# althonos/pyhmmer

Measured on AMD Instinct MI355X. Metric: GCUPS (DP cells/s) + seqs/s for hmmsearch, Pfam-A vs proteome, 1/2/4/8 GPUs, higher is better.
Workload: dtype u8/i16 filters (MSV, Viterbi), f32 Forward/Backward

## Files before the change

pyhmmer_amd/csrc/p7x_device.hpp:

```cpp
#pragma once
#include "p7x_internal.hpp"
#include "p7x_devmem.hpp"
#include <hip/hip_runtime.h>
#include <map>
#include <memory>
#include <mutex>

namespace p7x {

constexpr int kMaxL      = 100000;
constexpr int kTabRows   = 32;
constexpr int kNegPad    = -512;

#define P7X_HIP(call)                                                                          \
  do { hipError_t e_ = (call); if (e_ != hipSuccess) {                                         \
    p7x::set_error(std::string(#call) + ": " + hipGetErrorString(e_)); return e_ == hipErrorOutOfMemory ? P7X_EMEM : P7X_EDEVICE; } } while (0)

struct LengthTables {
  uint8_t *tjb = nullptr;
  int16_t *xwmove = nullptr;
  float   *null1 = nullptr;
  double  *logtab = nullptr;
};

struct DeviceCtx {
  int device = -1;
  hipStream_t stream = nullptr;
  hipStream_t stream2 = nullptr;
  LengthTables lt;
  int num_cu = 256;
  std::mutex mu;
  std::mutex msv_mu;
  std::mutex lt_scan_mu;
  static constexpr int kLtStreams = 4;
  hipStream_t lt_stream[kLtStreams]{};
  int lt_next = 0;
  hipEvent_t msv_done[2] = { nullptr, nullptr };
  int msv_last = -1;
  std::mutex slab_mu;
  std::multimap<size_t, void *> slab_free;
  size_t slab_free_bytes = 0;
  size_t slab_obtained_bytes = 0;
  static constexpr int kWsSets = 4, kWsSide = 7;
  hipStream_t ws_main[kWsSets]{};
  hipStream_t ws_side[kWsSets][kWsSide]{};
  std::vector<hipStream_t> ws_spacers;
  int ws_set_users[kWsSets]{};
};
int get_ctx(int device, DeviceCtx **out);
int create_tail_stream(DeviceCtx *ctx, bool high_priority, hipStream_t *out);

struct DevProfile {
  int device = -1;
  int M = 0, Kp = 0;
  int msvR = 0, msvK = 0, msvS = 0;
  uint32_t *msv_tab = nullptr;
  int16_t *msvw_emis = nullptr;
  uint32_t *msvw_pk = nullptr;
  int msvwC = 0, msvw_rows = kTabRows;
  int vitC = 0, Mpad = 0;
  int16_t *vit_trans = nullptr;
  int16_t *vit_emis = nullptr;
  int vitpkT = 0, vitpkP = 0;
  uint32_t *vitpk_trans = nullptr, *vitpk_emis = nullptr;
  float *fwd_trans = nullptr;
  float *fwd_emis = nullptr;
  int fwdgT = 0, fwdgC = 0;
  float *fwdg_trans = nullptr, *fwdg_emis = nullptr;
  float *bias_eo = nullptr;
  std::shared_ptr<DeviceBuf> shared;
};

int get_dev_profile(const p7x_oprofile *om, DeviceCtx *ctx, DevProfile **out);
int get_dev_profiles(const p7x_oprofile *const *oms, int n, DeviceCtx *ctx, DevProfile **out, int nthreads);
void free_dev_profile(DevProfile *d);

struct EnvelopeScorer;
struct EnsembleRunner;
}
struct p7x_seqdb;
#include <memory>
namespace p7x {
struct LongTargetWindowRegions;
int device_regions_of_all(const p7x_oprofile *om, const p7x_seqdb *db, std::vector<LongTargetWindowRegions> &out);
std::unique_ptr<EnvelopeScorer> make_device_envelope_scorer(DeviceCtx *ctx, const p7x_seqdb *db, float oa_guard);
std::unique_ptr<EnvelopeScorer> make_device_align_scorer(DeviceCtx *ctx, const p7x_seqdb *db, float oa_guard);
size_t align_budget_bytes();
std::unique_ptr<EnsembleRunner> make_device_ensemble_runner(DeviceCtx *ctx, const p7x_seqdb *db, float guard);

}

struct p7x_seqdb {
  int device = -1;
  int abc_type = 0, Kp = 0;
  int64_t n = 0;
  int64_t nres = 0;
  int64_t nslots = 0;
  int64_t ngroups = 0;
  std::vector<int32_t> h_len;
  std::vector<int32_t> h_order;
  std::vector<int64_t> h_off;
  std::vector<uint8_t> h_dsq;
  int64_t vit_long_slots = 0;
  std::vector<int32_t> h_grp_len;
  std::vector<int64_t> h_grp_suffix;
  uint8_t *d_dsq = nullptr;
  int64_t *d_slot_off = nullptr;
  int32_t *d_slot_len = nullptr;
  uint4   *d_tiles = nullptr;
  int64_t *d_grp_off = nullptr;
  int32_t *d_grp_nblk = nullptr;
  int64_t tile_u4 = 0;
  p7x::DeviceBuf slab;
};
```

pyhmmer_amd/csrc/p7x_devimage.hip:

```cpp
#include "p7x_device.hpp"
#include "p7x_kernels.hpp"
#include "p7x_host.hpp"
#include <cstring>
#include <memory>

namespace p7x {

static void chunk_transpose_fill(int M, int C, std::vector<int> &pos_of_node)
{
  pos_of_node.assign(M + 1, -1);
  for (int k = 1; k <= M; ++k) { const int z = (k - 1) / C, c = (k - 1) % C; pos_of_node[k] = c * 64 + z; }
}

void free_dev_profile(DevProfile *d)
{
  delete d;
}

struct DevCache { std::mutex mu; std::vector<DevProfile *> per_device; };

struct ImageStage { int device = -1; PinnedBuf pinned; hipStream_t stream = nullptr; };

struct HostImage {
  std::vector<char> bytes;
  std::vector<std::pair<void **, size_t>> fix;
  template <typename T, typename F>
  void add(F **field, const std::vector<T> &v)
  {
    const size_t off = bytes.size(), n = v.size() * sizeof(T);
    bytes.resize(((off + n + 255) / 256) * 256);
    std::memcpy(bytes.data() + off, v.data(), n);
    fix.emplace_back(reinterpret_cast<void **>(field), off);
  }
};

static void build_host_image(const Profile &p, DevProfile *d, HostImage &img)
{
  d->msvR = msv_pick(p.M, &d->msvK);
  if (d->msvR > 0) {
    d->msvS = msv_stride(d->msvR, d->msvK);
    std::vector<uint32_t> tab;
    msv_build_tables(p, d->msvR, d->msvK, tab);
    img.add(&d->msv_tab, tab);
  }
  d->vitC = vit_pick_C(p.M);
  if (d->vitC > 0) {
    const int C = d->vitC, Mpad = 64 * C, nrows = p.Kp + 1;
    d->Mpad = Mpad;
    std::vector<int> pos;
    chunk_transpose_fill(p.M, C, pos);
    std::vector<int16_t> vt((size_t) Mpad * 8, -32768), ve((size_t) nrows * Mpad, -32768);
    std::vector<float> ft((size_t) Mpad * 8, 0.0f), fe((size_t) nrows * Mpad, 0.0f);
    for (int k = 1; k <= p.M; ++k) {
      for (int t = 0; t < NTRANS; ++t) {
        vt[(size_t) pos[k] * 8 + t] = p.tw[(size_t) t * (p.M + 1) + k];
        ft[(size_t) pos[k] * 8 + t] = p.tf[(size_t) t * (p.M + 1) + k];
      }
      for (int x = 0; x < p.Kp; ++x) {
        ve[(size_t) x * Mpad + pos[k]] = p.rw[(size_t) x * (p.M + 1) + k];
        fe[(size_t) x * Mpad + pos[k]] = p.rf_[(size_t) x * (p.M + 1) + k];
      }
    }
    {
      std::vector<int16_t> me((size_t) kTabRows * Mpad, (int16_t) kNegPad);
      for (int k = 1; k <= p.M; ++k)
        for (int x = 0; x < p.Kp; ++x) me[(size_t) x * Mpad + pos[k]] = (int16_t) ((int) p.bias_b - (int) p.rb[(size_t) x * (p.M + 1) + k]);
      img.add(&d->msvw_emis, me);
      d->msvwC = C; d->msvw_rows = kTabRows;
      int Cp = 0;
      if ((d->msvR <= 0 || d->msvK >= 8) && C % 4 == 0 && C <= 32) Cp = C;
      else if (d->msvR <= 0 && C > 32 && p.M <= 2560 && p.Kp + 1 <= 30) { Cp = p.M <= 2304 ? 36 : 40; d->msvwC = Cp; d->msvw_rows = p.Kp + 1; }
      if (Cp > 0) {
        const int P2 = Cp / 4, rows = d->msvw_rows;
        std::vector<uint32_t> pk((size_t) rows * P2 * 64 * 2);
        auto em = [&](int x, int k) -> uint32_t { return (uint32_t) (uint16_t) (int16_t) ((x < p.Kp && k <= p.M) ? (int) p.bias_b - (int) p.rb[(size_t) x * (p.M + 1) + k] : kNegPad); };
        for (int x = 0; x < rows; ++x)
          for (int j2 = 0; j2 < P2; ++j2)
            for (int z = 0; z < 64; ++z)
              for (int h = 0; h < 2; ++h) {
                const int k = z * Cp + 2 * (2 * j2 + h) + 1;
                pk[(((size_t) x * P2 + j2) * 64 + z) * 2 + h] = em(x, k) | (em(x, k + 1) << 16);
              }
        img.add(&d->msvw_pk, pk);
      }
    }
    img.add(&d->vit_trans, vt);
    img.add(&d->vit_emis, ve);
    img.add(&d->fwd_trans, ft);
    img.add(&d->fwd_emis, fe);
    int gT = 0, gC = 0;
    if (fwdg_pick(p.M, d->vitC, &gT, &gC)) {
      std::vector<float> gt, ge;
      fwdg_build_tables(p, gT, gC, gt, ge);
      d->fwdgT = gT; d->fwdgC = gC;
      img.add(&d->fwdg_trans, gt);
      img.add(&d->fwdg_emis, ge);
    }
  }
  {
    int T = 0, P = 0;
    if (vitpk_pick(p.M, &T, &P)) {
      std::vector<uint32_t> tt, te;
      vitpk_build_tables(p, T, P, tt, te);
      d->vitpkT = T; d->vitpkP = P;
      img.add(&d->vitpk_trans, tt);
      img.add(&d->vitpk_emis, te);
    }
  }
  {
    const Alphabet &abc = Alphabet::get(p.abc_type);
    std::vector<float> eo((size_t) kTabRows * 2, 1.0f);
    for (int x = 0; x < p.K; ++x) { eo[x * 2 + 0] = p.bgf[x] / p.bgf[x]; eo[x * 2 + 1] = p.compo[x] / p.bgf[x]; }
    for (int x = p.K + 1; x <= p.Kp - 3; ++x)
      for (int s = 0; s < 2; ++s) {
        float e = 0.0f, den = 0.0f;
        for (int y = 0; y < p.K; ++y) if (abc.degen[x][y]) { e += (s == 0 ? p.bgf[y] : p.compo[y]); den += p.bgf[y]; }
        eo[x * 2 + s] = den > 0.0f ? e / den : 0.0f;
      }
    img.add(&d->bias_eo, eo);
  }
}

int get_dev_profiles(const p7x_oprofile *const *oms, int n, DeviceCtx *ctx, DevProfile **out, int nthreads)
{
  std::vector<int> missing;
  for (int i = 0; i < n; ++i) {
    out[i] = nullptr;
    auto *cache = static_cast<DevCache *>(oms[i]->dev_cache);
    std::lock_guard<std::mutex> lk(cache->mu);
    for (DevProfile *d : cache->per_device) if (d->device == ctx->device) { out[i] = d; break; }
    if (!out[i]) missing.push_back(i);
  }
  if (missing.empty()) return P7X_OK;
  const int nm = (int) missing.size();
  std::vector<std::unique_ptr<DevProfile>> fresh((size_t) nm);
  std::vector<HostImage> imgs((size_t) nm);
  auto build = [&](int z) {
    const Profile &p = oms[missing[(size_t) z]]->p;
    auto d = std::make_unique<DevProfile>();
    d->device = ctx->device; d->M = p.M; d->Kp = p.Kp;
    build_host_image(p, d.get(), imgs[(size_t) z]);
    fresh[(size_t) z] = std::move(d);
  };
  if (nm >= 4) host_parallel_for(nm, nthreads, build); else for (int z = 0; z < nm; ++z) build(z);
  std::vector<size_t> off((size_t) nm + 1, 0);
  for (int z = 0; z < nm; ++z) off[(size_t) z + 1] = off[(size_t) z] + imgs[(size_t) z].bytes.size();
  const size_t total = off[(size_t) nm];
  auto stage_lease = LeasePool<ImageStage>::instance().lease(ctx->device, [](const ImageStage &, const ImageStage *b) { return !b; });
  ImageStage &stg = *stage_lease;
  int st = P7X_OK;
  if ((st = stg.pinned.reserve(total, (size_t) 1 << 20)) != P7X_OK) return st;
  if (stg.stream == nullptr) P7X_HIP(hipStreamCreateWithFlags(&stg.stream, hipStreamNonBlocking));
  auto shared = std::make_shared<DeviceBuf>();
  if ((st = shared->reserve(ctx, total)) != P7X_OK) return st;
  char *const pinned = stg.pinned.as<char>(), *const slab = shared->as<char>();
  auto place = [&](int z) {
    const HostImage &img = imgs[(size_t) z];
    std::memcpy(pinned + off[(size_t) z], img.bytes.data(), img.bytes.size());
    for (const auto &f : img.fix) *f.first = slab + off[(size_t) z] + f.second;
    fresh[(size_t) z]->shared = shared;
  };
  if (nm >= 4) host_parallel_for(nm, nthreads, place); else for (int z = 0; z < nm; ++z) place(z);
  if (hipMemcpyAsync(slab, pinned, total, hipMemcpyHostToDevice, stg.stream) != hipSuccess ||
      hipStreamSynchronize(stg.stream) != hipSuccess) {
    set_error("uploading the profiles' device images failed");
    return P7X_EDEVICE;
  }
  for (int z = 0; z < nm; ++z) {
    const int i = missing[(size_t) z];
    auto *cache = static_cast<DevCache *>(oms[i]->dev_cache);
    std::lock_guard<std::mutex> lk(cache->mu);
    for (DevProfile *d : cache->per_device) if (d->device == ctx->device) { out[i] = d; break; }
    if (!out[i]) { out[i] = fresh[(size_t) z].get(); cache->per_device.push_back(fresh[(size_t) z].release()); }
  }
  return P7X_OK;
}

int get_dev_profile(const p7x_oprofile *om, DeviceCtx *ctx, DevProfile **out) { return get_dev_profiles(&om, 1, ctx, out, 1); }

}

using namespace p7x;

extern "C" {

void p7x_oprofile_destroy(p7x_oprofile *om)
// ... 14 lines not shown
```

pyhmmer_amd/csrc/p7x_kernels.hpp:

```cpp
#pragma once
#include <type_traits>
#include "p7x_device.hpp"

namespace p7x {

struct ArgRef { const void *base; uint32_t stride; };
#if defined(__HIPCC__)
template <class A> __device__ __forceinline__ A load_args(const ArgRef r)
{
#if defined(__HIP_DEVICE_COMPILE__)
  typedef const __attribute__((address_space(4))) A *cptr;
  return *(cptr) (unsigned long long) (static_cast<const char *>(r.base) + (size_t) blockIdx.y * r.stride);
#else
  return *reinterpret_cast<const A *>(static_cast<const char *>(r.base) + (size_t) blockIdx.y * r.stride);
#endif
}
#endif
template <class A> struct ArgRun {
  const A *host = nullptr; const void *dev = nullptr; uint32_t stride = 0; int n = 0;
  const A &at(int i) const { return *reinterpret_cast<const A *>(reinterpret_cast<const char *>(host) + (size_t) i * stride); }
  ArgRef ref() const { return ArgRef{ dev, stride }; }
};
inline unsigned lane_grid(long want, long resident, int nlanes)
{
  (void) nlanes;
  if (want > resident) want = resident;
  return (unsigned) (want < 1 ? 1 : want);
}

inline unsigned lane_grid_pull(long want, long resident, int nlanes, bool old_rule)
{
  if (old_rule || nlanes < 32) return lane_grid(want, resident, nlanes);
  long b = (2 * resident + nlanes - 1) / nlanes;
  if (b > resident) b = resident;
  if (b > want) b = want;
  return (unsigned) (b < 1 ? 1 : b);
}

struct MsvArgs {
  const uint32_t *tab;
  const uint4 *tiles;
  const int64_t *grp_off;
  const int32_t *grp_nblk;
  const int32_t *slot_len;
  const uint8_t *tjb_tab;
  int ngroups;
  int group_first;
  int base, bias, tec, tbm;
  int *counter;
  int16_t *out_xJ;
  int *amb_count; int *amb_groups; int *counter2;
  const int *group_list; const int *group_count;
  int R;
};
int  msv_pick(int M, int *K);
int  msv_stride(int R, int K);
void msv_build_tables(const Profile &p, int R, int K, std::vector<uint32_t> &out);
int  msv_launch(int R, int K, const ArgRun<MsvArgs> &main, const ArgRun<MsvArgs> *amb, int num_cu, hipStream_t st);
constexpr int kMsvTiers = 6;
int  msv_tier(int R, int K);
int  msv_tier_launch(int tier, const ArgRun<MsvArgs> &main, int num_cu, hipStream_t st);
int  msv_exact_launch(int R, int K, const ArgRun<MsvArgs> &amb, int num_cu, hipStream_t st);

#define P7X_NODE_TIERS(X) X(1) X(2) X(3) X(4) X(5) X(6) X(8) X(10) X(12) X(16) X(20) X(24) X(32) X(48) X(64) X(96) X(128)
template <class F> int node_tier_dispatch(int C, const char *too_long, F &&f)
{
  switch (C) {
#define P7X_TIER_CASE(CC) case CC: return f(std::integral_constant<int, CC>());
    P7X_NODE_TIERS(P7X_TIER_CASE)
#undef P7X_TIER_CASE
    default: set_error(too_long); return P7X_EINVAL;
  }
}
struct WaveSeqArgs {
  int M, C;
  const void *trans;
  const void *emis;
  const uint8_t *dsq;
  const int64_t *slot_off;
  const int32_t *slot_len;
  const int32_t *list;
  int nlist;
  const int *nlist_ptr;
  const int *abort_flag;
  int nrows;
  int *counter;
  const int16_t *xwmove_tab; int base_w, xw_e, ddbound;
  int32_t *out_xC;
  const int *lt_thresh;
  int *lt_nrec; int *lt_rec; int lt_cap;
  float xf_e_move, xf_e_loop;
  float *out_sc;
  float *xmx;
  const int64_t *xmx_off;
  const float *fwd_xmx;
};
int vit_pick_C(int M);
int vit_launch(const ArgRun<WaveSeqArgs> &a, int num_cu, hipStream_t st);
int fwd_launch(const ArgRun<WaveSeqArgs> &a, int num_cu, hipStream_t st);
bool fwdg_pick(int M, int vitC, int *T, int *C);
int fwdg_launch(const ArgRun<WaveSeqArgs> &a, int num_cu, hipStream_t st);
void fwdg_build_tables(const Profile &p, int T, int C, std::vector<float> &trans, std::vector<float> &emis);
int bck_launch(const ArgRun<WaveSeqArgs> &a, int num_cu, hipStream_t st);

struct MsvWaveArgs {
  int C, nrows;
  const void *emis;
  const void *emis_pk;
  const uint8_t *dsq; const int64_t *slot_off; const int32_t *slot_len; const uint8_t *tjb_tab;
  int nslots, base, bias, tec, tbm;
  int16_t *out_xJ;
};
int msv_wave_launch(const ArgRun<MsvWaveArgs> &a, int num_cu, hipStream_t st);

struct VitPkArgs {
  const void *trans, *emis;
  const uint8_t *dsq; const int64_t *slot_off; const int32_t *slot_len;
  const int32_t *list; int nlist; const int *nlist_ptr;
  const int *nskip_ptr;
  int nrows;
  const int16_t *xwmove_tab; int base_w, xw_e, ddbound;
  int32_t *out_xC;
};
bool vitpk_pick(int M, int *T, int *P);
void vitpk_build_tables(const Profile &p, int T, int P, std::vector<uint32_t> &trans, std::vector<uint32_t> &emis);
int  vitpk_launch(int T, int P, const ArgRun<VitPkArgs> &a, int num_cu, hipStream_t st);

struct EnvArgs {
  int M, C, K, nrows;
  const void *trans;
  const void *emis;
  const uint8_t *dsq;
  float nj, xf_e_move, xf_e_loop;
  int nenv;
  const int64_t *env_sq;
  const int32_t *env_len;
  const int32_t *env_L;
  const int32_t *order;
  int *cursor;
  float *work; int64_t work_stride; int Lmax;
  int nblocks, slab_base;
  float *out_sc;
  const float *env_emis;
  long long env_emis_stride;
  float *out_orig;
  float oa_guard;
  int32_t *out_status;
  float *out_null2;
  const int64_t *tr_off;
  uint32_t *tr_a; int32_t *tr_i; float *tr_pp;
  int32_t *tr_n;
};
constexpr int env_waves(int C) { return C >= 8 ? 4 : 8; }
enum class EnvMode { Envelope, LongTarget, Align };
inline size_t env_work_floats(int C, int Lmax)
{
  const size_t rows = (size_t) Lmax + 1, Mpad = (size_t) 64 * C;
  size_t f = 2 * rows * Mpad + rows * (6 + 6 + 5 + 3 + 1);
  f += (rows * Mpad + 1) / 2;
  return (f + 63) & ~(size_t) 63;
}
int env_max_blocks(EnvMode mode, int C, int nrows, int num_cu, int *nblocks);
int env_launch(EnvMode mode, const ArgRun<EnvArgs> &a, hipStream_t st);
__host__ __device__ inline float align_pp_guard(int M) { return 1.0e-5f + 2.5e-9f * (float) M; }
__host__ __device__ inline float align_pp_band(int M) { return 0.5f - 10.0f * align_pp_guard(M); }
int align_max_blocks(int C, int nrows, int num_cu, int *nblocks);
int align_launch(const ArgRun<EnvArgs> &a, hipStream_t st);

struct ChoiceCell; struct ChoiceRow;
struct EnsRegion {
  int64_t sq;
  int64_t cell0;
  int64_t row0;
  int64_t dom0;
  int32_t Lr, L;
  int32_t job, dom_cap;
};
struct EnsJob {
  int M, C, K, Kp, nrows, Q;
  const void *trans, *emis;
  const float *rft;
  const uint8_t *degen;
  int reg_first, nreg;
};
struct EnsArgs {
  const EnsJob *jobs; const EnsRegion *regions; int nregions;
  const uint8_t *dsq;
  ChoiceCell *cells; float2 *md; ChoiceRow *rows;
  uint32_t seed_x;
  int nsamples;
  float *n2acc;
  int32_t *dom;
  int32_t *out_ndom; int32_t *out_status;
  int lds_bytes;
  uint32_t guard;
};

struct SsvLongArgs {
  const uint32_t *tab4q;
  const uint32_t *tab_full;
  const uint8_t *dsq;
  const uint8_t *comp;
  int pair_slack;
  const long long *chunk_list;
  long long L;
  int M, Kp;
  int chunk_len;
  long long chunks_per_strand, nchunks;
// ... 12 lines not shown
```

pyhmmer_amd/csrc/p7x_pipeline.hip:

```cpp
#include "p7x_wave.hpp"
#include "p7x_host.hpp"
#include <atomic>
#include <chrono>
#include <cmath>
#include <cstdlib>
#include <cstring>
#include <memory>
#include <string>

namespace p7x {

struct StageBufs {
  int16_t *xJ;
  float *usc, *filtersc, *vfsc, *fwdsc;
  int32_t *xC;
  float *fwd_by_item;
  int32_t *list_bias, *list_vit, *list_fwd, *list_fin;
  uint8_t *stage;
  int *counters;
};

struct StageParams {
  double F1, F2, F3;
  double F3_near;
// ... 556 lines not shown
static ListEstimates estimate_lists(const p7x_pipeline_cfg &cfg, int64_t nslots)
{
  auto est = [&](double f, double slack, int floor_) {
    const double v = cfg.do_max ? (double) nslots : std::min<double>((double) nslots, (double) nslots * f * slack + floor_);
    return (int) std::min<double>(v, (double) INT_MAX);
  };
  ListEstimates e;
  e.bias = est(cfg.F1, 2.0, 1024); e.vit = e.bias;
  e.fwd = est(cfg.F2, 8.0, 512);
  e.fin = est(cfg.F3, 50.0, 1024);
  return e;
}

static WaveSeqArgs ws_args(const Profile &p, const DevProfile *dp, const p7x_seqdb *db, DeviceCtx *ctx)
{
  WaveSeqArgs a{};
  a.M = p.M; a.C = dp->vitC; a.nrows = p.Kp + 1;
  a.dsq = db->d_dsq; a.slot_off = db->d_slot_off; a.slot_len = db->d_slot_len;
  a.xwmove_tab = ctx->lt.xwmove; a.base_w = p.base_w; a.xw_e = p.xw[XE][MOVE]; a.ddbound = p.ddbound_w;
  a.xf_e_move = p.xf[XE][MOVE]; a.xf_e_loop = p.xf[XE][LOOP];
  return a;
}

static bool msv_exact_only() { return debug_opt(OPT_MSV_EXACT) > 0; }
static bool vit_wave_only() { return debug_opt(OPT_VIT_WAVE) > 0; }
static bool device_clustered(int host_threads)
{
  const int forced = debug_opt(OPT_DEVICE_CLUSTERED);
  if (forced >= 0) return forced != 0;
  const int threads = host_threads > 0 ? std::min(host_threads, tophits_usable_cpus()) : tophits_usable_cpus();
  return threads < 12;
}

static bool small_block(const p7x_seqdb *db, const DeviceCtx *ctx, int nlanes)
{
  return debug_opt(OPT_SMALL_BLOCK) != 0 && db->ngroups * (int64_t) nlanes <= (int64_t) ctx->num_cu * 4;
}

static int long_groups(const p7x_seqdb *db, const DeviceCtx *ctx, int nlanes)
{
  if (debug_opt(OPT_MSV_LONG_GROUPS) == 0 || db->ngroups < 2) return 0;
  const int64_t resident = (int64_t) ctx->num_cu * 4 * 3;
  const int64_t G = db->ngroups;
  int64_t g = 0;
  while (g < G / 2 && (int64_t) db->h_grp_len[(size_t) g] * resident > (int64_t) nlanes * db->h_grp_suffix[(size_t) g]) ++g;
  return (int) g;
}

static void fill_msv_args(LaneArgs &la, const Profile &p, const DevProfile *dp, const p7x_seqdb *db, DeviceCtx *ctx, const StageBufs &b,
                          int nlong = 0)
{
  MsvWaveArgs w{};
  w.C = dp->msvwC; w.nrows = dp->msvw_rows; w.emis = dp->msvw_emis; w.emis_pk = dp->msvw_pk; w.dsq = db->d_dsq; w.slot_off = db->d_slot_off; w.slot_len = db->d_slot_len;
  w.tjb_tab = ctx->lt.tjb; w.nslots = (int) db->nslots; w.base = p.base_b; w.bias = p.bias_b; w.tec = p.tec_b; w.tbm = p.tbm_b;
  w.out_xJ = b.xJ;
  if (nlong > 0) w.nslots = (int) std::min<int64_t>((int64_t) nlong * 64, db->nslots);
  la.msvw = w;
  MsvArgs a{};
  a.group_first = nlong;
  a.tab = dp->msv_tab; a.tiles = db->d_tiles; a.grp_off = db->d_grp_off; a.grp_nblk = db->d_grp_nblk;
  a.slot_len = db->d_slot_len; a.tjb_tab = ctx->lt.tjb; a.ngroups = (int) db->ngroups;
  a.base = p.base_b; a.bias = p.bias_b; a.tec = p.tec_b; a.tbm = p.tbm_b;
  a.counter = &b.counters[0]; a.out_xJ = b.xJ;
  a.amb_count = &b.counters[10]; a.counter2 = &b.counters[11];
  a.amb_groups = msv_exact_only() ? nullptr : b.list_fin;
  a.R = dp->msvR;
  la.msv = a;
  MsvArgs x = a;
  x.group_list = a.amb_groups; x.group_count = a.amb_count; x.counter = a.counter2; x.amb_groups = nullptr;
  la.msv_amb = x;
}

static void fill_vit_args(LaneArgs &la, const Profile &p, const DevProfile *dp, const p7x_seqdb *db, DeviceCtx *ctx,
                          const int32_t *list, int nlist, const int *nlist_ptr, int32_t *out_xC,
                          const int *nlong_ptr = nullptr, int nlong_bound = 0)
{
  WaveSeqArgs w = ws_args(p, dp, db, ctx);
  w.trans = dp->vit_trans; w.emis = dp->vit_emis; w.list = list; w.nlist = nlist; w.nlist_ptr = nlist_ptr; w.out_xC = out_xC;
  if (nlong_ptr) { w.nlist_ptr = nlong_ptr; w.nlist = nlong_bound; }
  la.vit = w;
  VitPkArgs a{};
  a.trans = dp->vitpk_trans; a.emis = dp->vitpk_emis; a.dsq = db->d_dsq; a.slot_off = db->d_slot_off; a.slot_len = db->d_slot_len;
  a.list = list; a.nlist = nlist; a.nlist_ptr = nlist_ptr; a.nskip_ptr = nlong_ptr; a.nrows = p.Kp + 1;
  a.xwmove_tab = ctx->lt.xwmove; a.base_w = p.base_w; a.xw_e = p.xw[XE][MOVE]; a.ddbound = p.ddbound_w;
  a.out_xC = out_xC;
  la.vitpk = a;
}

template <class A> static ArgRun<A> lane_run(const Workspace *ws, A LaneArgs::*member, int first, int n)
{
  ArgRun<A> r;
  r.host = &(ws->h_args.as<LaneArgs>()[first].*member);
  r.dev = reinterpret_cast<const char *>(ws->d_args.as<LaneArgs>() + first) + (reinterpret_cast<const char *>(r.host) - reinterpret_cast<const char *>(ws->h_args.as<LaneArgs>() + first));
  r.stride = (uint32_t) sizeof(LaneArgs); r.n = n;
  return r;
}

struct LaneModel { const p7x_oprofile *om = nullptr; DevProfile *dp = nullptr; };

static int upload_args(Workspace *ws, int first, int n, hipStream_t s)
{
  P7X_HIP(hipMemcpyAsync(ws->d_args.as<LaneArgs>() + first, ws->h_args.as<LaneArgs>() + first, (size_t) n * sizeof(LaneArgs), hipMemcpyHostToDevice, s));
  return P7X_OK;
}

struct LaneClass { int first = 0, n = 0; long msv_key = 0, vit_key = 0; int C = 0; int nlong = 0; int64_t vit_long = 0; };

static long msv_key_of(const DevProfile *dp, bool small)
{
  return (dp->msvR <= 0 || small) ? -(long) dp->msvwC : (long) (dp->msvK * 1000 + dp->msvR);
}
static long vit_key_of(const DevProfile *dp, bool small)
{
  return (dp->vitpkT > 0 && !vit_wave_only() && !small) ? (long) (dp->vitpkT * 256 + dp->vitpkP) : -(long) dp->vitC;
}

static int lane_classes(const std::vector<LaneModel> &lm, const p7x_seqdb *db, const DeviceCtx *ctx, std::vector<LaneClass> &out)
{
  const int nl = (int) lm.size();
  const bool small = small_block(db, ctx, nl);
  const int nlong = small ? 0 : long_groups(db, ctx, nl);
  out.clear();
  for (int l = 0; l < nl; ++l) {
    const DevProfile *dp = lm[l].dp;
    if ((dp->msvR <= 0 || small) && !dp->msvw_emis) { set_error("model too long for the MSV kernels (M > 8192)"); return P7X_EINVAL; }
    LaneClass c; c.first = l; c.n = 1; c.msv_key = msv_key_of(dp, small); c.vit_key = vit_key_of(dp, small); c.C = dp->vitC;
    c.nlong = (c.msv_key >= 0 && dp->msvw_emis) ? nlong : 0;
    c.vit_long = c.vit_key >= 0 ? db->vit_long_slots : 0;
    if (!out.empty() && out.back().msv_key == c.msv_key && out.back().vit_key == c.vit_key && out.back().C == c.C) out.back().n++;
    else out.push_back(c);
  }
  return P7X_OK;
}

static int class_msv(const LaneClass &c, const std::vector<LaneModel> &lm, DeviceCtx *ctx, Workspace *ws, hipStream_t stream)
{
  if (c.msv_key < 0) return msv_wave_launch(lane_run(ws, &LaneArgs::msvw, c.first, c.n), ctx->num_cu, stream);
  if (c.nlong > 0) {
    const int st = msv_wave_launch(lane_run(ws, &LaneArgs::msvw, c.first, c.n), ctx->num_cu, stream);
    if (st != P7X_OK) return st;
  }
  const ArgRun<MsvArgs> amb = lane_run(ws, &LaneArgs::msv_amb, c.first, c.n);
  return msv_launch(lm[c.first].dp->msvR, lm[c.first].dp->msvK, lane_run(ws, &LaneArgs::msv, c.first, c.n), msv_exact_only() ? nullptr : &amb, ctx->num_cu, stream);
}

static int class_msv_rest(const LaneClass &c, const std::vector<LaneModel> &lm, DeviceCtx *ctx, Workspace *ws, hipStream_t stream)
{
  if (c.nlong > 0) {
    const int st = msv_wave_launch(lane_run(ws, &LaneArgs::msvw, c.first, c.n), ctx->num_cu, stream);
    if (st != P7X_OK) return st;
  }
  return msv_exact_launch(lm[c.first].dp->msvR, lm[c.first].dp->msvK, lane_run(ws, &LaneArgs::msv_amb, c.first, c.n), ctx->num_cu, stream);
}
static bool msv_tiers_enabled() { return !msv_exact_only() && debug_opt(OPT_MSV_F16) != 0 && debug_opt(OPT_MSV_TIERS) != 0; }

static int class_viterbi(const LaneClass &c, const std::vector<LaneModel> &lm, DeviceCtx *ctx, Workspace *ws, hipStream_t s)
{
  if (c.vit_key < 0) return vit_launch(lane_run(ws, &LaneArgs::vit, c.first, c.n), ctx->num_cu, s);
  if (c.vit_long > 0) {
    const int st = vit_launch(lane_run(ws, &LaneArgs::vit, c.first, c.n), ctx->num_cu, s);
    if (st != P7X_OK) return st;
  }
  return vitpk_launch(lm[c.first].dp->vitpkT, lm[c.first].dp->vitpkP, lane_run(ws, &LaneArgs::vitpk, c.first, c.n), ctx->num_cu, s);
}

static int class_wave(const LaneClass &c, Workspace *ws, WaveSeqArgs LaneArgs::*member, bool backward, DeviceCtx *ctx, hipStream_t s)
{
// ... 1086 lines not shown
```

pyhmmer_amd/csrc/p7x_vitpk.hip:

```cpp
#include <map>
#include "p7x_wave.hpp"
#include <mutex>

namespace p7x {

namespace {

typedef short s2v __attribute__((ext_vector_type(2)));
__device__ __forceinline__ s2v as_s2v(uint32_t u) { return __builtin_bit_cast(s2v, u); }
__device__ __forceinline__ uint32_t as_u(s2v v) { return __builtin_bit_cast(uint32_t, v); }
__device__ __forceinline__ uint32_t pk_adds(uint32_t a, uint32_t b) { return as_u(__builtin_elementwise_add_sat(as_s2v(a), as_s2v(b))); }
__device__ __forceinline__ uint32_t pk_max(uint32_t a, uint32_t b) { return as_u(__builtin_elementwise_max(as_s2v(a), as_s2v(b))); }
__device__ __forceinline__ uint32_t splat16(int v) { const uint32_t w = (uint32_t) v & 0xffffu; return w | (w << 16); }
__device__ __forceinline__ int lo_of(uint32_t w) { return (int) (short) (w & 0xffffu); }
__device__ __forceinline__ int hi_of(uint32_t w) { return (int) (short) (w >> 16); }

constexpr uint32_t kNeg2 = 0x80008000u;
constexpr int vitpk_rowq(int T, int P)
{
  const int n = ((P + 3) / 4) * T;
  return T == 8 ? ((n & 15) == 8 ? n : n + 8) : n;
}

#define P7X_DPP_U(v, ctrl) ((uint32_t) __builtin_amdgcn_update_dpp((int) kNeg2, (int) (v), (ctrl), 0xf, 0xf, false))

template <int T>
__device__ __forceinline__ int group_max(uint32_t v)
{
  v = pk_max(v, P7X_DPP_U(v, 0xB1));
  v = pk_max(v, P7X_DPP_U(v, 0x4E));
  v = pk_max(v, P7X_DPP_U(v, 0x141));
  if constexpr (T == 16) v = pk_max(v, P7X_DPP_U(v, 0x140));
  return max(lo_of(v), hi_of(v));
}

}

struct RowState { int xN, xB, xJ, xC; bool overflow; };

template <int T>
__device__ __forceinline__ uint32_t stripe_shift(uint32_t r, bool first)
{
  const uint32_t prev = P7X_DPP_U(r, 0x138);
  const uint32_t last = P7X_DPP_U(r, T == 8 ? 0x141 : 0x140);
  return first ? ((last << 16) | 0x8000u) : prev;
}

template <int T, int P>
__device__ __forceinline__ void vit_row(const VitPkArgs &a, const uint4 *tral, const uint4 *trbl, const uint4 *er, bool first,
                                        bool active, int xwm, const uint32_t (&mi)[P], const uint32_t (&ii)[P],
                                        const uint32_t (&di)[P], uint32_t (&mo_)[P], uint32_t (&io_)[P], uint32_t (&do_)[P],
                                        const uint32_t (&tdd)[P], RowState &rs)
{
  constexpr int PS = (P + 3) & ~3;
  const uint32_t xBv = splat16(rs.xB);
  uint32_t mp = stripe_shift<T>(mi[P - 1], first), ip = stripe_shift<T>(ii[P - 1], first), dp = stripe_shift<T>(di[P - 1], first);
  uint32_t xEv = kNeg2, dmaxv = kNeg2, dcv = kNeg2;
#pragma unroll
  for (int j4 = 0; j4 < PS; j4 += 4) {
    const uint4 e4 = er[(j4 / 4) * T];
    const uint32_t ev[4] = { e4.x, e4.y, e4.z, e4.w };
#pragma unroll
    for (int jj = 0; jj < 4; ++jj) {
      const int q = j4 + jj;
      if (q < P) {
        const uint4 ta = tral[q * T], tb = trbl[q * T];
        const uint32_t a0 = pk_adds(xBv, ta.x), a1 = pk_adds(mp, ta.y), a2 = pk_adds(ip, ta.z), a3 = pk_adds(dp, ta.w);
        uint32_t sv = pk_max(pk_max(a0, a1), pk_max(a2, a3));
        sv = pk_adds(sv, ev[jj]);
        xEv = pk_max(xEv, sv);
        mo_[q] = sv;
        if (q > 0) do_[q] = dcv;
        dcv = pk_adds(sv, tb.x);
        dmaxv = pk_max(dmaxv, dcv);
        io_[q] = pk_max(pk_adds(mi[q], tb.y), pk_adds(ii[q], tb.z));
        mp = mi[q]; ip = ii[q]; dp = di[q];
      }
    }
    asm volatile("" ::: "memory");
  }
  do_[0] = stripe_shift<T>(dcv, first);
  const int xE = group_max<T>(xEv);
  const int Dmax = group_max<T>(dmaxv);
  if (active) {
    if (xE >= 32767) rs.overflow = true;
    rs.xC = max(rs.xC, xE + a.xw_e);
    rs.xJ = max(rs.xJ, xE + a.xw_e);
    rs.xB = max(rs.xJ + xwm, rs.xN + xwm);
  }
  const bool trig = active && (Dmax + a.ddbound > rs.xB);
#ifdef P7X_VITPK_NO_CLOSURE
  if (false) {
#else
  if (__any(trig)) {
#endif
    int pass = 0;
    bool more;
    do {
#pragma unroll
      for (int q = 1; q < P; ++q) do_[q] = pk_max(do_[q], pk_adds(do_[q - 1], tdd[q - 1]));
      uint32_t c = stripe_shift<T>(pk_adds(do_[P - 1], tdd[P - 1]), first);
      if (!trig) c = kNeg2;
      const uint32_t d0 = pk_max(do_[0], c);
      const bool changed = d0 != do_[0];
      do_[0] = d0;
      more = __any(changed) && ++pass < 2 * T;
    } while (more);
  }
}

template <int T, int P>
__global__ void __launch_bounds__(256) vitpk_kernel(const ArgRef ref)
{
  constexpr int G = 64 / T;
  const VitPkArgs a = load_args<VitPkArgs>(ref);
  const int nlist = a.nlist_ptr ? *a.nlist_ptr : a.nlist;
  const int nskip = a.nskip_ptr ? *a.nskip_ptr : 0;
  if (nskip + (int) (blockIdx.x * 4 * G) >= nlist) return;
  constexpr int PS = (P + 3) & ~3;
  constexpr int ROWQ = vitpk_rowq(T, P);
  extern __shared__ __attribute__((aligned(16))) unsigned char smem[];
  uint4 *tra = reinterpret_cast<uint4 *>(smem);
  uint4 *trb = tra + P * T;
  uint4 *em = trb + P * T;
  {
    const uint4 *gt = reinterpret_cast<const uint4 *>(a.trans);
    for (int i = threadIdx.x; i < 2 * P * T; i += 256) tra[i] = gt[i];
    const uint4 *ge = reinterpret_cast<const uint4 *>(a.emis);
    for (int i = threadIdx.x; i < a.nrows * ROWQ; i += 256) em[i] = ge[i];
  }
  __syncthreads();
  const int lane = threadIdx.x & 63;
  const int s = lane % T, g = lane / T;
  const bool first = (s == 0);
  const int wave0 = rfl((int) (blockIdx.x * 4 + (threadIdx.x >> 6)));
  const int nwaves = (int) gridDim.x * 4;
  const uint4 *tral = tra + s, *trbl = trb + s, *eml = em + s;
  uint32_t tdd[P];
#pragma unroll
  for (int q = 0; q < P; ++q) tdd[q] = trbl[q * T].w;

  for (int it0 = nskip + wave0 * G; it0 < nlist; it0 += nwaves * G) {
    const int it = it0 + g;
    const bool have = it < nlist;
    const int slot = have ? (a.list ? a.list[it] : it) : 0;
    const int L = have ? a.slot_len[slot] : 0;
    const uint8_t *sq = a.dsq + (have ? a.slot_off[slot] : 0);
    const int xwm = (int) a.xwmove_tab[L];
    const int Lmax = wave_max_i32(L);

    uint32_t mA[P], iA[P], dA[P], mB[P], iB[P], dB[P];
#pragma unroll
    for (int j = 0; j < P; ++j) mA[j] = iA[j] = dA[j] = kNeg2;
    RowState rs;
    rs.xN = a.base_w; rs.xB = rs.xN + xwm; rs.xJ = -32768; rs.xC = -32768; rs.overflow = false;

    for (int i0 = 0; i0 < Lmax; i0 += 4 * T) {
      uint32_t word = 0;
#pragma unroll
      for (int b = 0; b < 4; ++b) {
        const int r = i0 + 4 * s + b;
        const uint32_t x = (r < L) ? (uint32_t) sq[r] : 0u;
        word |= x << (8 * b);
      }
      const int nrow = min(4 * T, Lmax - i0);
      auto residue = [&](int r) -> uint32_t {
        const uint32_t w = (uint32_t) __shfl((int) word, g * T + (r >> 2));
        return (w >> (8 * (r & 3))) & 0xffu;
      };
      int r = 0;
      for (; r + 1 < nrow; r += 2) {
        vit_row<T, P>(a, tral, trbl, eml + residue(r) * ROWQ, first, i0 + r < L, xwm, mA, iA, dA, mB, iB, dB, tdd, rs);
        vit_row<T, P>(a, tral, trbl, eml + residue(r + 1) * ROWQ, first, i0 + r + 1 < L, xwm, mB, iB, dB, mA, iA, dA, tdd, rs);
      }
      if (r < nrow) {
        vit_row<T, P>(a, tral, trbl, eml + residue(r) * ROWQ, first, i0 + r < L, xwm, mA, iA, dA, mB, iB, dB, tdd, rs);
#pragma unroll
        for (int j = 0; j < P; ++j) { mA[j] = mB[j]; iA[j] = iB[j]; dA[j] = dB[j]; }
      }
    }
    const bool overflow = rs.overflow; const int xC = rs.xC;
    if (have && s == 0) a.out_xC[it] = overflow ? 32767 : xC;
  }
}

bool vitpk_pick(int M, int *T, int *P)
{
  static const int p8[] = { 2, 4, 6, 8, 10, 12, 14, 15, 16, 17, 18, 19, 20 };
  static const int p16[] = { 11, 12, 13, 14, 15, 16, 17, 18, 19, 20 };
  for (int p : p8) if (M <= 8 * 2 * p) { *T = 8; *P = p; return true; }
  for (int p : p16) if (M <= 16 * 2 * p) { *T = 16; *P = p; return true; }
  return false;
}

void vitpk_build_tables(const Profile &p, int T, int P, std::vector<uint32_t> &trans, std::vector<uint32_t> &emis)
{
  const int rowq = vitpk_rowq(T, P), nrows = p.Kp + 1;
  auto pack = [](int lo, int hi) { return ((uint32_t) lo & 0xffffu) | (((uint32_t) hi & 0xffffu) << 16); };
  trans.assign((size_t) 2 * P * T * 4, kNeg2);
  emis.assign((size_t) nrows * rowq * 4, kNeg2);
  for (int s = 0; s < T; ++s)
    for (int j = 0; j < P; ++j) {
      const int k0 = s * P + j + 1, k1 = (s + T) * P + j + 1;
      for (int t = 0; t < NTRANS; ++t) {
        const int lo = (k0 <= p.M) ? p.tw[(size_t) t * (p.M + 1) + k0] : -32768;
        const int hi = (k1 <= p.M) ? p.tw[(size_t) t * (p.M + 1) + k1] : -32768;
        trans[((size_t) (t / 4) * P * T + (size_t) j * T + s) * 4 + (t % 4)] = pack(lo, hi);
      }
      for (int x = 0; x < p.Kp; ++x) {
        const int lo = (k0 <= p.M) ? p.rw[(size_t) x * (p.M + 1) + k0] : -32768;
        const int hi = (k1 <= p.M) ? p.rw[(size_t) x * (p.M + 1) + k1] : -32768;
        emis[((size_t) x * rowq + (size_t) (j / 4) * T + s) * 4 + (j % 4)] = pack(lo, hi);
      }
    }
}

template <int T, int P>
static int launch_pk(const ArgRun<VitPkArgs> &a, int num_cu, hipStream_t st)
{
  const size_t lds = ((size_t) 2 * P * T + (size_t) a.at(0).nrows * vitpk_rowq(T, P)) * 16;
  auto kern = vitpk_kernel<T, P>;
  static std::map<int, int> per_cu_by_device;
  static std::mutex mu;
  int per_cu = 0;
  {
    int dev = 0; P7X_HIP(hipGetDevice(&dev));
    std::lock_guard<std::mutex> lk(mu);
    int &cached = per_cu_by_device[dev];
    if (cached == 0) {
      if (lds > 64 * 1024) P7X_HIP(hipFuncSetAttribute(reinterpret_cast<const void *>(kern), hipFuncAttributeMaxDynamicSharedMemorySize, (int) lds));
      P7X_HIP(hipOccupancyMaxActiveBlocksPerMultiprocessor(&cached, kern, 256, lds));
      if (cached < 1) cached = 1;
    }
    per_cu = cached;
  }
  long want = 0;
  for (int i = 0; i < a.n; ++i) want = std::max<long>(want, ((long) a.at(i).nlist + 4 * (64 / T) - 1) / (4 * (64 / T)));
  if (want <= 0) return P7X_OK;
  hipLaunchKernelGGL(kern, dim3(lane_grid(want, (long) num_cu * per_cu, a.n), (unsigned) a.n), dim3(256), lds, st, a.ref());
  P7X_HIP(hipGetLastError());
  return P7X_OK;
}

int vitpk_launch(int T, int P, const ArgRun<VitPkArgs> &a, int num_cu, hipStream_t st)
{
  if (a.n <= 0) return P7X_OK;
#define P7X_PK(TT, PP) if (T == TT && P == PP) return launch_pk<TT, PP>(a, num_cu, st);
  P7X_PK(8, 2) P7X_PK(8, 4) P7X_PK(8, 6) P7X_PK(8, 8) P7X_PK(8, 10) P7X_PK(8, 12) P7X_PK(8, 14) P7X_PK(8, 15) P7X_PK(8, 16)
  P7X_PK(8, 17) P7X_PK(8, 18) P7X_PK(8, 19) P7X_PK(8, 20)
  P7X_PK(16, 11) P7X_PK(16, 12) P7X_PK(16, 13) P7X_PK(16, 14) P7X_PK(16, 15) P7X_PK(16, 16) P7X_PK(16, 17) P7X_PK(16, 18)
  P7X_PK(16, 19) P7X_PK(16, 20)
#undef P7X_PK
  set_error("no packed Viterbi kernel for this model length");
  return P7X_EINVAL;
}

}
```

Baseline: 24470.

## Hoist begin terms, keep transitions in registers, bound D-closure trigger via max MD

```diff
diff --git a/pyhmmer_amd/csrc/p7x_device.hpp b/pyhmmer_amd/csrc/p7x_device.hpp
--- a/pyhmmer_amd/csrc/p7x_device.hpp
+++ b/pyhmmer_amd/csrc/p7x_device.hpp
@@ -61,7 +61,7 @@
   int vitC = 0, Mpad = 0;
   int16_t *vit_trans = nullptr;
   int16_t *vit_emis = nullptr;
-  int vitpkT = 0, vitpkP = 0;
+  int vitpkT = 0, vitpkP = 0, vitpk_mdmax = -32768;
   uint32_t *vitpk_trans = nullptr, *vitpk_emis = nullptr;
   float *fwd_trans = nullptr;
   float *fwd_emis = nullptr;
diff --git a/pyhmmer_amd/csrc/p7x_devimage.hip b/pyhmmer_amd/csrc/p7x_devimage.hip
--- a/pyhmmer_amd/csrc/p7x_devimage.hip
+++ b/pyhmmer_amd/csrc/p7x_devimage.hip
@@ -101,7 +101,7 @@
     int T = 0, P = 0;
     if (vitpk_pick(p.M, &T, &P)) {
       std::vector<uint32_t> tt, te;
-      vitpk_build_tables(p, T, P, tt, te);
+      vitpk_build_tables(p, T, P, tt, te, &d->vitpk_mdmax);
       d->vitpkT = T; d->vitpkP = P;
       img.add(&d->vitpk_trans, tt);
       img.add(&d->vitpk_emis, te);
diff --git a/pyhmmer_amd/csrc/p7x_kernels.hpp b/pyhmmer_amd/csrc/p7x_kernels.hpp
--- a/pyhmmer_amd/csrc/p7x_kernels.hpp
+++ b/pyhmmer_amd/csrc/p7x_kernels.hpp
@@ -86,6 +86,7 @@
   int nrows;
   int *counter;
   const int16_t *xwmove_tab; int base_w, xw_e, ddbound;
+  int mdmax;
   int32_t *out_xC;
   const int *lt_thresh;
   int *lt_nrec; int *lt_rec; int lt_cap;
@@ -120,10 +121,11 @@
   const int *nskip_ptr;
   int nrows;
   const int16_t *xwmove_tab; int base_w, xw_e, ddbound;
+  int mdmax;
   int32_t *out_xC;
 };
 bool vitpk_pick(int M, int *T, int *P);
-void vitpk_build_tables(const Profile &p, int T, int P, std::vector<uint32_t> &trans, std::vector<uint32_t> &emis);
+void vitpk_build_tables(const Profile &p, int T, int P, std::vector<uint32_t> &trans, std::vector<uint32_t> &emis, int *mdmax);
 int  vitpk_launch(int T, int P, const ArgRun<VitPkArgs> &a, int num_cu, hipStream_t st);
 
 struct EnvArgs {
diff --git a/pyhmmer_amd/csrc/p7x_pipeline.hip b/pyhmmer_amd/csrc/p7x_pipeline.hip
--- a/pyhmmer_amd/csrc/p7x_pipeline.hip
+++ b/pyhmmer_amd/csrc/p7x_pipeline.hip
@@ -662,7 +662,7 @@
   VitPkArgs a{};
   a.trans = dp->vitpk_trans; a.emis = dp->vitpk_emis; a.dsq = db->d_dsq; a.slot_off = db->d_slot_off; a.slot_len = db->d_slot_len;
   a.list = list; a.nlist = nlist; a.nlist_ptr = nlist_ptr; a.nskip_ptr = nlong_ptr; a.nrows = p.Kp + 1;
-  a.xwmove_tab = ctx->lt.xwmove; a.base_w = p.base_w; a.xw_e = p.xw[XE][MOVE]; a.ddbound = p.ddbound_w;
+  a.xwmove_tab = ctx->lt.xwmove; a.base_w = p.base_w; a.xw_e = p.xw[XE][MOVE]; a.ddbound = p.ddbound_w; a.mdmax = dp->vitpk_mdmax;
   a.out_xC = out_xC;
   la.vitpk = a;
 }
diff --git a/pyhmmer_amd/csrc/p7x_vitpk.hip b/pyhmmer_amd/csrc/p7x_vitpk.hip
--- a/pyhmmer_amd/csrc/p7x_vitpk.hip
+++ b/pyhmmer_amd/csrc/p7x_vitpk.hip
@@ -46,16 +46,34 @@
   return first ? ((last << 16) | 0x8000u) : prev;
 }
 
+#ifndef P7X_VITPK_REGTRANS_MAXP
+#define P7X_VITPK_REGTRANS_MAXP 10
+#endif
+constexpr bool vitpk_regtrans(int P) { return P <= P7X_VITPK_REGTRANS_MAXP; }
+constexpr int vitpk_ntreg(int P) { return vitpk_regtrans(P) ? 6 * P : 1; }
+
+template <int T, int P>
+__device__ __forceinline__ void begin_terms(const uint4 *trbl, int xB, uint32_t (&bm)[P])
+{
+  const uint32_t xBv = splat16(xB);
+#pragma unroll
+  for (int q = 0; q < P; ++q) bm[q] = pk_adds(xBv, trbl[q * T].w);
+}
+
 template <int T, int P>
 __device__ __forceinline__ void vit_row(const VitPkArgs &a, const uint4 *tral, const uint4 *trbl, const uint4 *er, bool first,
                                         bool active, int xwm, const uint32_t (&mi)[P], const uint32_t (&ii)[P],
                                         const uint32_t (&di)[P], uint32_t (&mo_)[P], uint32_t (&io_)[P], uint32_t (&do_)[P],
-                                        const uint32_t (&tdd)[P], RowState &rs)
+                                        const uint32_t (&tdd)[P], const uint32_t (&treg)[vitpk_ntreg(P)], uint32_t (&bm)[P],
+                                        RowState &rs)
 {
   constexpr int PS = (P + 3) & ~3;
-  const uint32_t xBv = splat16(rs.xB);
+  constexpr bool RT = vitpk_regtrans(P);
   uint32_t mp = stripe_shift<T>(mi[P - 1], first), ip = stripe_shift<T>(ii[P - 1], first), dp = stripe_shift<T>(di[P - 1], first);
-  uint32_t xEv = kNeg2, dmaxv = kNeg2, dcv = kNeg2;
+  uint32_t xEv = kNeg2, dcv = kNeg2;
+#ifdef P7X_VITPK_EXACT_DMAX
+  uint32_t dmaxv = kNeg2;
+#endif
 #pragma unroll
   for (int j4 = 0; j4 < PS; j4 += 4) {
     const uint4 e4 = er[(j4 / 4) * T];
@@ -64,16 +82,25 @@
     for (int jj = 0; jj < 4; ++jj) {
       const int q = j4 + jj;
       if (q < P) {
-        const uint4 ta = tral[q * T], tb = trbl[q * T];
-        const uint32_t a0 = pk_adds(xBv, ta.x), a1 = pk_adds(mp, ta.y), a2 = pk_adds(ip, ta.z), a3 = pk_adds(dp, ta.w);
-        uint32_t sv = pk_max(pk_max(a0, a1), pk_max(a2, a3));
+        uint32_t tMM, tIM, tDM, tMD, tMI, tII;
+        if constexpr (RT) {
+          tMM = treg[6 * q]; tIM = treg[6 * q + 1]; tDM = treg[6 * q + 2]; tMD = treg[6 * q + 3]; tMI = treg[6 * q + 4]; tII = treg[6 * q + 5];
+        } else {
+          const uint4 ta = tral[q * T];
+          const uint2 tb = *reinterpret_cast<const uint2 *>(trbl + q * T);
+          tMM = ta.x; tIM = ta.y; tDM = ta.z; tMD = ta.w; tMI = tb.x; tII = tb.y;
+        }
+        const uint32_t a1 = pk_adds(mp, tMM), a2 = pk_adds(ip, tIM), a3 = pk_adds(dp, tDM);
+        uint32_t sv = pk_max(pk_max(bm[q], a1), pk_max(a2, a3));
         sv = pk_adds(sv, ev[jj]);
         xEv = pk_max(xEv, sv);
         mo_[q] = sv;
         if (q > 0) do_[q] = dcv;
-        dcv = pk_adds(sv, tb.x);
+        dcv = pk_adds(sv, tMD);
+#ifdef P7X_VITPK_EXACT_DMAX
         dmaxv = pk_max(dmaxv, dcv);
-        io_[q] = pk_max(pk_adds(mi[q], tb.y), pk_adds(ii[q], tb.z));
+#endif
+        io_[q] = pk_max(pk_adds(mi[q], tMI), pk_adds(ii[q], tII));
         mp = mi[q]; ip = ii[q]; dp = di[q];
       }
     }
@@ -81,14 +108,21 @@
   }
   do_[0] = stripe_shift<T>(dcv, first);
   const int xE = group_max<T>(xEv);
-  const int Dmax = group_max<T>(dmaxv);
+  bool moved = false;
   if (active) {
     if (xE >= 32767) rs.overflow = true;
     rs.xC = max(rs.xC, xE + a.xw_e);
     rs.xJ = max(rs.xJ, xE + a.xw_e);
-    rs.xB = max(rs.xJ + xwm, rs.xN + xwm);
-  }
-  const bool trig = active && (Dmax + a.ddbound > rs.xB);
+    const int xB = max(rs.xJ + xwm, rs.xN + xwm);
+    moved = xB != rs.xB;
+    rs.xB = xB;
+  }
+  if (__any(moved)) begin_terms<T, P>(trbl, rs.xB, bm);
+#ifdef P7X_VITPK_EXACT_DMAX
+  const bool trig = active && (group_max<T>(dmaxv) + a.ddbound > rs.xB);
+#else
+  const bool trig = active && (max(xE + a.mdmax, -32768) + a.ddbound > rs.xB);
+#endif
 #ifdef P7X_VITPK_NO_CLOSURE
   if (false) {
 #else
@@ -138,7 +172,15 @@
   const uint4 *tral = tra + s, *trbl = trb + s, *eml = em + s;
   uint32_t tdd[P];
 #pragma unroll
-  for (int q = 0; q < P; ++q) tdd[q] = trbl[q * T].w;
+  for (int q = 0; q < P; ++q) tdd[q] = trbl[q * T].z;
+  uint32_t treg[vitpk_ntreg(P)];
+  if constexpr (vitpk_regtrans(P)) {
+#pragma unroll
+    for (int q = 0; q < P; ++q) {
+      const uint4 ta = tral[q * T], tb = trbl[q * T];
+      treg[6 * q] = ta.x; treg[6 * q + 1] = ta.y; treg[6 * q + 2] = ta.z; treg[6 * q + 3] = ta.w; treg[6 * q + 4] = tb.x; treg[6 * q + 5] = tb.y;
+    }
+  } else treg[0] = 0;
 
   for (int it0 = nskip + wave0 * G; it0 < nlist; it0 += nwaves * G) {
     const int it = it0 + g;
@@ -154,6 +196,8 @@
     for (int j = 0; j < P; ++j) mA[j] = iA[j] = dA[j] = kNeg2;
     RowState rs;
     rs.xN = a.base_w; rs.xB = rs.xN + xwm; rs.xJ = -32768; rs.xC = -32768; rs.overflow = false;
+    uint32_t bm[P];
+    begin_terms<T, P>(trbl, rs.xB, bm);
 
     for (int i0 = 0; i0 < Lmax; i0 += 4 * T) {
       uint32_t word = 0;
@@ -170,11 +214,11 @@
       };
       int r = 0;
       for (; r + 1 < nrow; r += 2) {
-        vit_row<T, P>(a, tral, trbl, eml + residue(r) * ROWQ, first, i0 + r < L, xwm, mA, iA, dA, mB, iB, dB, tdd, rs);
-        vit_row<T, P>(a, tral, trbl, eml + residue(r + 1) * ROWQ, first, i0 + r + 1 < L, xwm, mB, iB, dB, mA, iA, dA, tdd, rs);
+        vit_row<T, P>(a, tral, trbl, eml + residue(r) * ROWQ, first, i0 + r < L, xwm, mA, iA, dA, mB, iB, dB, tdd, treg, bm, rs);
+        vit_row<T, P>(a, tral, trbl, eml + residue(r + 1) * ROWQ, first, i0 + r + 1 < L, xwm, mB, iB, dB, mA, iA, dA, tdd, treg, bm, rs);
       }
       if (r < nrow) {
-        vit_row<T, P>(a, tral, trbl, eml + residue(r) * ROWQ, first, i0 + r < L, xwm, mA, iA, dA, mB, iB, dB, tdd, rs);
+        vit_row<T, P>(a, tral, trbl, eml + residue(r) * ROWQ, first, i0 + r < L, xwm, mA, iA, dA, mB, iB, dB, tdd, treg, bm, rs);
 #pragma unroll
         for (int j = 0; j < P; ++j) { mA[j] = mB[j]; iA[j] = iB[j]; dA[j] = dB[j]; }
       }
@@ -184,35 +228,54 @@
   }
 }
 
+#ifdef P7X_VITPK_EVEN_TILES
+#define P7X_VITPK_TILES(X) \
+  X(8, 2) X(8, 4) X(8, 6) X(8, 8) X(8, 10) X(8, 12) X(8, 14) X(8, 15) X(8, 16) \
+  X(8, 17) X(8, 18) X(8, 19) X(8, 20) \
+  X(16, 11) X(16, 12) X(16, 13) X(16, 14) X(16, 15) X(16, 16) X(16, 17) X(16, 18) X(16, 19) X(16, 20)
+#else
+#define P7X_VITPK_TILES(X) \
+  X(8, 2) X(8, 3) X(8, 4) X(8, 5) X(8, 6) X(8, 7) X(8, 8) X(8, 9) X(8, 10) X(8, 11) X(8, 12) X(8, 13) X(8, 14) X(8, 15) X(8, 16) \
+  X(8, 17) X(8, 18) X(8, 19) X(8, 20) \
+  X(16, 11) X(16, 12) X(16, 13) X(16, 14) X(16, 15) X(16, 16) X(16, 17) X(16, 18) X(16, 19) X(16, 20)
+#endif
+
 bool vitpk_pick(int M, int *T, int *P)
 {
-  static const int p8[] = { 2, 4, 6, 8, 10, 12, 14, 15, 16, 17, 18, 19, 20 };
-  static const int p16[] = { 11, 12, 13, 14, 15, 16, 17, 18, 19, 20 };
-  for (int p : p8) if (M <= 8 * 2 * p) { *T = 8; *P = p; return true; }
-  for (int p : p16) if (M <= 16 * 2 * p) { *T = 16; *P = p; return true; }
+#define P7X_PK(TT, PP) if (M <= 2 * TT * PP) { *T = TT; *P = PP; return true; }
+  P7X_VITPK_TILES(P7X_PK)
+#undef P7X_PK
   return false;
 }
 
-void vitpk_build_tables(const Profile &p, int T, int P, std::vector<uint32_t> &trans, std::vector<uint32_t> &emis)
+void vitpk_build_tables(const Profile &p, int T, int P, std::vector<uint32_t> &trans, std::vector<uint32_t> &emis, int *mdmax)
 {
   const int rowq = vitpk_rowq(T, P), nrows = p.Kp + 1;
   auto pack = [](int lo, int hi) { return ((uint32_t) lo & 0xffffu) | (((uint32_t) hi & 0xffffu) << 16); };
   trans.assign((size_t) 2 * P * T * 4, kNeg2);
   emis.assign((size_t) nrows * rowq * 4, kNeg2);
+  auto lo_of_host = [](uint32_t w) { return (int) (int16_t) (w & 0xffffu); };
+  auto hi_of_host = [](uint32_t w) { return (int) (int16_t) (w >> 16); };
+  int md_max = -32768;
   for (int s = 0; s < T; ++s)
     for (int j = 0; j < P; ++j) {
       const int k0 = s * P + j + 1, k1 = (s + T) * P + j + 1;
+      static const int word_of[NTRANS] = { 7, 0, 1, 2, 3, 4, 5, 6 };
       for (int t = 0; t < NTRANS; ++t) {
         const int lo = (k0 <= p.M) ? p.tw[(size_t) t * (p.M + 1) + k0] : -32768;
         const int hi = (k1 <= p.M) ? p.tw[(size_t) t * (p.M + 1) + k1] : -32768;
-        trans[((size_t) (t / 4) * P * T + (size_t) j * T + s) * 4 + (t % 4)] = pack(lo, hi);
-      }
+        const int w = word_of[t];
+        trans[((size_t) (w / 4) * P * T + (size_t) j * T + s) * 4 + (w % 4)] = pack(lo, hi);
+      }
+      const uint32_t md = trans[((size_t) j * T + s) * 4 + 3];
+      md_max = std::max(md_max, std::max(lo_of_host(md), hi_of_host(md)));
       for (int x = 0; x < p.Kp; ++x) {
         const int lo = (k0 <= p.M) ? p.rw[(size_t) x * (p.M + 1) + k0] : -32768;
         const int hi = (k1 <= p.M) ? p.rw[(size_t) x * (p.M + 1) + k1] : -32768;
         emis[((size_t) x * rowq + (size_t) (j / 4) * T + s) * 4 + (j % 4)] = pack(lo, hi);
       }
     }
+  *mdmax = md_max;
 }
 
 template <int T, int P>
@@ -246,10 +309,7 @@
 {
   if (a.n <= 0) return P7X_OK;
 #define P7X_PK(TT, PP) if (T == TT && P == PP) return launch_pk<TT, PP>(a, num_cu, st);
-  P7X_PK(8, 2) P7X_PK(8, 4) P7X_PK(8, 6) P7X_PK(8, 8) P7X_PK(8, 10) P7X_PK(8, 12) P7X_PK(8, 14) P7X_PK(8, 15) P7X_PK(8, 16)
-  P7X_PK(8, 17) P7X_PK(8, 18) P7X_PK(8, 19) P7X_PK(8, 20)
-  P7X_PK(16, 11) P7X_PK(16, 12) P7X_PK(16, 13) P7X_PK(16, 14) P7X_PK(16, 15) P7X_PK(16, 16) P7X_PK(16, 17) P7X_PK(16, 18)
-  P7X_PK(16, 19) P7X_PK(16, 20)
+  P7X_VITPK_TILES(P7X_PK)
 #undef P7X_PK
   set_error("no packed Viterbi kernel for this model length");
   return P7X_EINVAL;
```

Measured after the change: 23740. 0.97x the previous value.
